# CERALIVE/ceracoder

Hardware: AMD Instinct MI355X
Metric: 1080p H.264 encoded frames/sec per GPU (higher is better)
Workload: dtype u8

## Files before the change

ceracoder_amd/csrc/k_deblock.hip:

```cpp
#include "intra_mb.hpp"

DEV void filter_line(const dev_tables *T, uint8_t *pix, int step, int bS, int qp_p, int qp_q, bool chroma) {
    if (bS == 0) return;
    const int idx = clip3(0, 51, (qp_p + qp_q + 1) >> 1);
    const int alpha = T->alpha[idx], beta = T->beta[idx];
    const int p0 = pix[-step], p1 = pix[-2 * step], q0 = pix[0], q1 = pix[step];
    if (!(iabs(p0 - q0) < alpha && iabs(p1 - p0) < beta && iabs(q1 - q0) < beta)) return;
    if (chroma) {
        if (bS < 4) {
            const int tc = T->tc0[idx][bS - 1] + 1;
            const int dl = clip3(-tc, tc, (((q0 - p0) << 2) + (p1 - q1) + 4) >> 3);
            pix[-step] = (uint8_t)clip255(p0 + dl); pix[0] = (uint8_t)clip255(q0 - dl);
        } else {
            pix[-step] = (uint8_t)((2 * p1 + p0 + q1 + 2) >> 2); pix[0] = (uint8_t)((2 * q1 + q0 + p1 + 2) >> 2);
        }
        return;
    }
    const int p2 = pix[-3 * step], q2 = pix[2 * step];
    const bool ap = iabs(p2 - p0) < beta, aq = iabs(q2 - q0) < beta;
    if (bS < 4) {
        const int tc0 = T->tc0[idx][bS - 1];
        const int tc = tc0 + (ap ? 1 : 0) + (aq ? 1 : 0);
        const int dl = clip3(-tc, tc, (((q0 - p0) << 2) + (p1 - q1) + 4) >> 3);
        pix[-step] = (uint8_t)clip255(p0 + dl); pix[0] = (uint8_t)clip255(q0 - dl);
// ... 228 lines not shown
}
DEV void edge_chroma2(const edge_par &P, int p1, int &p0, int &q0, int q1, int bS) {
    const bool f = (bS != 0) & (adiff(p0, q0) < P.alpha) & (adiff(p1, p0) < P.beta) & (adiff(q1, q0) < P.beta);
    const int tc = (int)((P.tc0 >> (8 * ((bS - 1) & 3))) & 0xFF) + 1;
    const int dl = clip3(-tc, tc, (((q0 - p0) << 2) + (p1 - q1) + 4) >> 3);
    const bool s4 = bS == 4;
    const int sp0 = (2 * p1 + p0 + q1 + 2) >> 2, sq0 = (2 * q1 + q0 + p1 + 2) >> 2, wp0 = clip255(p0 + dl), wq0 = clip255(q0 - dl);
    const int np0 = s4 ? sp0 : wp0, nq0 = s4 ? sq0 : wq0;
    p0 = f ? np0 : p0; q0 = f ? nq0 : q0;
}

DEV int quad_prev(int v) { return __builtin_amdgcn_update_dpp(0, v, 0x90, 0xF, 0xF, false); }
DEV int quad_next(int v) { return __builtin_amdgcn_update_dpp(0, v, 0xF9, 0xF, 0xF, false); }
#define DBT_NB 8
struct dbt_luma { uint8_t t[DBT_NB][256]; uint8_t up[DBT_NB][64]; unsigned par[4][32]; };
struct dbt_chroma { uint8_t t[DBT_NB][128]; uint8_t up[DBT_NB][32]; unsigned par[4][32]; };
DEV uint4 lds128(const void *p) { return *(const uint4 *)p; }

template <bool ALL_INTRA>
DEV void edges4p_luma(const int e, const unsigned par, const bool any4, int *s) {
    int bS = (int)(par & 15u);
    const int alpha = (int)((par >> 8) & 255u), beta = (int)((par >> 16) & 255u), tc0 = (int)(par >> 24);
    if (ALL_INTRA || any4) {
        edge_par PE; PE.alpha = alpha; PE.beta = beta; PE.tc0 = (unsigned)tc0 * 0x010101u;
        edge_luma2<true>(PE, s[0], s[1], s[2], s[3], s[4], s[5], s[6], s[7], e == 0 ? bS : 0, true);
        const int f1 = quad_prev(s[5]), f2 = quad_prev(s[6]);
        s[1] = e == 1 ? f1 : s[1]; s[2] = e == 1 ? f2 : s[2];
        bS = e == 0 ? 0 : bS;
    }
    const int p1 = s[2], p0 = s[3], q0 = s[4], q1 = s[5], q2 = s[6];
    const int mf = ((adiff(p0, q0) - alpha) & (adiff(p1, p0) - beta) & (adiff(q1, q0) - beta) & -bS) >> 31;
// ... 9 lines not shown
    const int np1 = p1 + clip3(-tc0, tc0, (p2 + avg - (p1 << 1)) >> 1);
    s[3] = bsel(mf, clip255(p0 + dl), p0); s[4] = bsel(mf, clip255(q0 - dl), q0);
    s[2] = bsel(mf & map, np1, p1); s[5] = q1f;
}
DEV void edge_chroma_p(const unsigned par, int p1, int &p0, int &q0, int q1) {
    const int bS = (int)(par & 15u), alpha = (int)((par >> 8) & 255u), beta = (int)((par >> 16) & 255u), tc = (int)(par >> 24) + 1;
    const bool f = (bS != 0) & (adiff(p0, q0) < alpha) & (adiff(p1, p0) < beta) & (adiff(q1, q0) < beta);
    const int dl = clip3(-tc, tc, (((q0 - p0) << 2) + (p1 - q1) + 4) >> 3);
    const bool s4 = bS == 4;
    const int sp0 = (2 * p1 + p0 + q1 + 2) >> 2, sq0 = (2 * q1 + q0 + p1 + 2) >> 2, wp0 = clip255(p0 + dl), wq0 = clip255(q0 - dl);
    const int np0 = s4 ? sp0 : wp0, nq0 = s4 ? sq0 : wq0;
    p0 = f ? np0 : p0; q0 = f ? nq0 : q0;
}
DEV unsigned par_word(unsigned nib, unsigned ab, unsigned tcw) { return nib | (ab << 8) | (((tcw >> (8 * ((nib - 1) & 3))) & 255u) << 24); }

template <bool CHROMA, bool ALL_INTRA, int ROWS, bool GATED>
DEV void rows3_body(const db_args &a, const int band, const int nb, uint8_t *lds, const int part) {
    constexpr int rows_mb = CHROMA ? 8 : 16, strip = CHROMA ? 2 : 4, ring_n = CHROMA ? 8 : 16;
    constexpr int ROW_LDS = CHROMA ? (int)sizeof(dbt_chroma) : (int)sizeof(dbt_luma);
    constexpr int TILE = rows_mb * 16, UPB = strip * 16;
    const frame_ctx_t *__restrict__ ctx = &a.ctx;
    const int mbw = ctx->mbw, mbh = ctx->mbh, stride = ctx->stride;
    const int wid = __builtin_amdgcn_readfirstlane(threadIdx.x >> 6), lane = threadIdx.x & 63;
    const int role = wid / ROWS, r = wid - role * ROWS;
    const int my = band * ROWS + r;
    const bool row_ok = my < mbh, last_row = my == mbh - 1 || db_slice_last(ctx, my), dbtop = db_has_top(ctx, my);
    const bool fed = row_ok && r == 0 && dbtop;
    const bool feeds = row_ok && r == ROWS - 1 && !last_row;
    if (!ALL_INTRA && a.row_done) {
        if (threadIdx.x < 64) {
            const int r = (band - 1) * ROWS - 1 + (int)threadIdx.x;
            const bool mine = (int)threadIdx.x < 3 * ROWS + 1 && r >= 0 && r < mbh;
            const unsigned *w = a.row_done + (mine ? r * MI355_PROG_STRIDE : 0);
            int spins = 0;
            while (__ballot(mine && (int)(ld_sc1(w) - a.row_need) < 0)) {
                __builtin_amdgcn_s_sleep(8);
                if (++spins > DB_SPIN_MAX) { st_sc1(a.err, 17u | ((unsigned)band << 8) | (CHROMA ? 0x8000u : 0u)); break; }
                if ((spins & 1023) == 0 && ld_sc1(a.err)) break;
            }
            __builtin_amdgcn_fence(__ATOMIC_ACQUIRE, "agent");
            asm volatile("s_waitcnt vmcnt(0)" ::: "memory");
        }
        __syncthreads();
    }
    if (ALL_INTRA && a.iband_done) {
        if (threadIdx.x == 0) {
            const unsigned tag = ~ctx->epoch;
            const int r_lo = band * ROWS > 0 ? band * ROWS - 1 : 0, r_hi = band * ROWS + ROWS - 1 < mbh ? band * ROWS + ROWS - 1 : mbh - 1;
            int spins = 0;
            for (int ib = r_lo / a.ib_rows; ib <= r_hi / a.ib_rows; ib++)
                while (ld_sc1(a.iband_done + ib) != tag) {
                    __builtin_amdgcn_s_sleep(8);
                    if (++spins > DB_SPIN_MAX) { st_sc1(a.err, 11u); break; } if ((spins & 1023) == 0 && ld_sc1(a.err)) { break; }
                }
            __builtin_amdgcn_fence(__ATOMIC_ACQUIRE, "agent");
            asm volatile("s_waitcnt vmcnt(0)" ::: "memory");
        }
        __syncthreads();
    }
    if (a.qpc) {
        if (threadIdx.x == 0) {
            const unsigned need = a.qpc_base + (unsigned)((band + 1) * ROWS < mbh ? (band + 1) * ROWS : mbh);
            int spins = 0;
            while ((int)(ld_sc1(a.qpc) - need) < 0) {
                __builtin_amdgcn_s_sleep(8);
                if (++spins > DB_SPIN_MAX) { st_sc1(a.err, 23u | ((unsigned)band << 8)); break; }
                if ((spins & 1023) == 0 && ld_sc1(a.err)) break;
            }
            __builtin_amdgcn_fence(__ATOMIC_ACQUIRE, "agent");
            asm volatile("s_waitcnt vmcnt(0)" ::: "memory");
        }
        __syncthreads();
    }
#ifdef TL_PROF
    if (!CHROMA && threadIdx.x == 0) { const int sl = band == 0 ? 9 : band == nb / 2 ? 11 : band == nb - 1 ? 13 : -1; if (sl >= 0) *((volatile unsigned long long *)ctx->dbrec + (ctx->epoch & 63) * 16 + sl) = wall_clock64(); }
#endif
    constexpr int PARW = CHROMA ? 16 : 32;
    unsigned *partab = a.partab + (CHROMA ? (size_t)nb * ROWS * mbw * 32 : 0) + (size_t)band * ROWS * mbw * PARW;
    unsigned *flagw = (unsigned *)(lds + ROWS * ROW_LDS);
    unsigned *firsti = flagw + 4;
    unsigned *busyw = firsti + ROWS;
    if (threadIdx.x < 3) flagw[threadIdx.x] = 0;
    if (threadIdx.x < 2) busyw[threadIdx.x] = 0;
    if (GATED && threadIdx.x < ROWS) firsti[threadIdx.x] = (unsigned)mbw;
    const int cut_mid = mbw >> 1, cut_w = (mbw >> 2) < 31 ? (mbw >> 2) : 31;
    __syncthreads();
    {
        const dev_tables *T = &g_tab;
        const int per = ROWS * mbw;
        for (int j = threadIdx.x; j < per; j += 192 * ROWS) {
            const int row = band * ROWS + j / mbw;
            if (row < mbh) {
                unsigned w[16], pw[PARW];
                const bool work = db_record(ctx, T, j % mbw, row, w);
                if (GATED && (ldg32(&ctx->mbi[(size_t)row * mbw + j % mbw].mb_type) & 255u) != 1u) atomicMin(&firsti[j / mbw], (unsigned)(j % mbw));
#pragma unroll
                for (int d = 0; d < 2; d++)
#pragma unroll
                    for (int ed = 0; ed < (CHROMA ? 2 : 4); ed++)
#pragma unroll
                        for (int sg = 0; sg < 4; sg++) {
                            unsigned nib, ab, tc;
                            if (!CHROMA) {
                                nib = (w[2 * d + (ed >> 1)] >> (16 * (ed & 1) + 4 * sg)) & 15u;
                                ab = ed == 0 ? w[4 + 2 * d] : w[8]; tc = ed == 0 ? w[5 + 2 * d] : w[9];
                            } else {
                                nib = (w[2 * d + ed] >> (4 * sg)) & 15u;
                                ab = ed == 0 ? w[10 + 2 * d] : w[14]; tc = ed == 0 ? w[11 + 2 * d] : w[15];
                            }
                            pw[d * (PARW / 2) + ed * 4 + sg] = par_word(nib, ab, tc);
                        }
#pragma unroll
                for (int q = 0; q < PARW / 4; q++) stg128(partab + (size_t)j * PARW + 4 * q, make_uint4(pw[4 * q], pw[4 * q + 1], pw[4 * q + 2], pw[4 * q + 3]));
                if (work) flagw[1] = 1u;
                if (part >= 0) {
                    const int kc = j % mbw - (cut_mid - cut_w);
                    if (kc >= 0 && kc <= 2 * cut_w && ((pw[0] | pw[1] | pw[2] | pw[3]) & 15u) != 0) atomicOr(&busyw[kc >> 5], 1u << (kc & 31));
                }
            }
        }
#ifdef TL_PROF
        if (!CHROMA && band == 0 && threadIdx.x == 0) *((volatile unsigned long long *)ctx->dbrec + (ctx->epoch & 63) * 16 + 14) = wall_clock64();
#endif
        if (!ALL_INTRA) {
            for (int i = threadIdx.x; i < 2 * per; i += 192 * ROWS) {
                const int which = i < per ? 0 : 2, j = i < per ? i : i - per;
                const int row = (band - 1 + which) * ROWS + j / mbw;
                if (row >= 0 && row < mbh) {
                    const mb_info_t m = ld_mbinfo(&ctx->mbi[(size_t)row * mbw + j % mbw]);
                    if (m.mb_type != 1 || (m.nzmask & 0xFFFFu) != 0) flagw[which] = 1u;
                }
            }
            __syncthreads();
            for (int which = 0; which < 3; which += 2)
                if (flagw[which] == 0)
                    for (int j = threadIdx.x; j < per; j += 192 * ROWS) {
                        const int row = (band - 1 + which) * ROWS + j / mbw;
                        unsigned w[16];
                        if (row >= 0 && row < mbh && db_record(ctx, T, j % mbw, row, w)) flagw[which] = 1u;
                    }
        }
    }
    asm volatile("s_waitcnt vmcnt(0)" ::: "memory");
    __syncthreads();
    auto publish = [&](const bool drained) {
        if (!a.band_done) return;
        if (!drained) { asm volatile("s_waitcnt vmcnt(0)" ::: "memory"); __syncthreads(); }
        if (part >= 0) {
            if (threadIdx.x == 0) {
                __builtin_amdgcn_fence(__ATOMIC_RELEASE, "agent");
                asm volatile("s_waitcnt vmcnt(0)" ::: "memory");
                flagw[3] = __hip_atomic_fetch_add(a.part_cnt + 2 * band + (CHROMA ? 1 : 0), 1u, __ATOMIC_RELAXED, __HIP_MEMORY_SCOPE_AGENT) & 1u;
            }
            __syncthreads();
            if (flagw[3] == 0) return;
        }
        if (threadIdx.x < DB_DONE_COPIES) {
            __builtin_amdgcn_fence(__ATOMIC_RELEASE, "agent");
            asm volatile("s_waitcnt vmcnt(0)" ::: "memory");
            st_sc1(a.band_done + DB_DONE_STRIDE * threadIdx.x + 2 * band + (CHROMA ? 1 : 0), ctx->epoch);
        }
    };
    uint2 *cutg = part >= 0 ? (uint2 *)(a.part_cnt + 2 * nb) + 2 * band + (CHROMA ? 1 : 0) : nullptr;
    if (!ALL_INTRA && flagw[1] == 0) {
        if (cutg && threadIdx.x == 0) st64_sc1(cutg, make_uint2(0u, ctx->epoch));
        publish(true);
        return;
    }
    int x0 = 0, x1 = mbw;
    if (part >= 0) {
        int cut = mbw;
        int cut_up = 0;
        if (!ALL_INTRA && db_has_top(ctx, band * ROWS) && flagw[0] != 0) {
            if (threadIdx.x == 0) {
                uint2 g;
                int spins = 0;
                while ((g = ld64_sc1(cutg - 2)).y != ctx->epoch) {
                    __builtin_amdgcn_s_sleep(4);
                    if (++spins > DB_SPIN_MAX) { st_sc1(a.err, 24u | ((unsigned)band << 8) | (CHROMA ? 0x8000u : 0u)); g.x = 0; break; }
                    if ((spins & 1023) == 0 && ld_sc1(a.err)) { g.x = 0; break; }
                }
                flagw[3] = g.x;
            }
            __syncthreads();
            cut_up = (int)flagw[3];
            __syncthreads();
        }
        if (!ALL_INTRA && mbw >= 16) {
            int tgt = cut_w - (cut_w >> 3);
            const int lo = (cut_up > 0 && cut_up < mbw) ? cut_up - (cut_mid - cut_w) : 0;
            tgt = tgt > lo ? tgt : lo;
            const unsigned long long busy = (unsigned long long)busyw[0] | ((unsigned long long)busyw[1] << 32);
            for (int d = 0; d <= 2 * cut_w && cut == mbw; d++) {
                if (tgt + d <= 2 * cut_w && !((busy >> (tgt + d)) & 1ull)) cut = cut_mid - cut_w + tgt + d;
                else if (tgt - d >= lo && tgt - d >= 0 && !((busy >> (tgt - d)) & 1ull)) cut = cut_mid - cut_w + tgt - d;
            }
        }
        cut = __builtin_amdgcn_readfirstlane(cut);
        if (threadIdx.x == 0) st64_sc1(cutg, make_uint2((unsigned)cut, ctx->epoch));
        if (part == 0) x1 = cut; else x0 = cut;
        if (x0 >= x1) { publish(true); return; }
    }
#ifdef TL_PROF
    if (!CHROMA && band == 0 && threadIdx.x == 0) *((volatile unsigned long long *)ctx->dbrec + (ctx->epoch & 63) * 16 + 15) = wall_clock64();
#endif
    const bool up_work = ALL_INTRA || flagw[0] != 0;
    const bool dn_work = ALL_INTRA || flagw[2] != 0;
    const unsigned epoch = ctx->epoch;
    uint2 *gran_up = a.gran + (CHROMA ? (size_t)nb * mbw * 16 : 0) + (size_t)(band > 0 ? band - 1 : 0) * mbw * ring_n;
    uint2 *gran_my = a.gran + (CHROMA ? (size_t)nb * mbw * 16 : 0) + (size_t)band * mbw * ring_n;
    uint8_t *__restrict__ plane = CHROMA ? ctx->rec_uv : ctx->rec_y;
    const size_t row0 = (size_t)my * rows_mb;
    uint8_t *rowl = lds + r * ROW_LDS;
    uint8_t *tiles = rowl;
    uint8_t *ups = rowl + DBT_NB * TILE;
    unsigned *pars = (unsigned *)(rowl + DBT_NB * (TILE + UPB));
    uint8_t *tiles_up = lds + (r > 0 ? r - 1 : 0) * ROW_LDS;
    const int keep = last_row ? rows_mb : rows_mb - strip;
    const int t_end = (x1 - x0) + ROWS + 1;
    const int k = lane >> 2, e = lane & 3;
    uint4 preA, preB;
    uint2 gA, gB;
    const bool rlane = lane < rows_mb, uplane = lane >= 16 && lane < 16 + strip, glane = lane >= 32 && lane < 32 + ring_n;
    const int my_c = row_ok ? my : mbh - 1;
    constexpr int PL = PARW / 4;
    const bool plane_l = lane >= 16 && lane < 16 + PL;
// ... 9 lines not shown
    unsigned nmiss = 0;
#define DBT_TICK(i) do { tm1 = __builtin_readcyclecounter(); pc[i] += tm1 - tm0; tm0 = tm1; } while (0)
#define DBT_T0() tm0 = __builtin_readcyclecounter()
#else
#define DBT_TICK(i) do { } while (0)
#define DBT_T0() do { } while (0)
#endif
    const int t_last = t_end | 1;
    if (role == 0) {
        for (int t = -2; t <= t_last; t++) {
            DBT_T0();
            const int x = x0 + t - 1 - r;
            const bool act = row_ok && x >= x0 && x < x1;
                uint8_t *tile = tiles + (x & (DBT_NB - 1)) * TILE;
                if (act) {
                    const unsigned par = pars[(x & 3) * PARW + (CHROMA ? (lane & 1) * 4 + (lane >> 3) : e * 4 + (k >> 2))];
                    if (!CHROMA) {
                        uint8_t *tl = tiles + ((x - 1) & (DBT_NB - 1)) * TILE;
                        unsigned *pw = (unsigned *)(e == 0 ? tl + k * 16 + 12 : tile + k * 16 + 4 * e - 4), *qw = (unsigned *)(tile + k * 16 + 4 * e);
                        const unsigned w0 = *pw, w1 = *qw;
                        const unsigned long long work = __ballot((par & 15u) != 0);
                        if (ALL_INTRA || work) {
                            int s[8];
#pragma unroll
                            for (int i = 0; i < 4; i++) { s[i] = byte_of(w0, i); s[4 + i] = byte_of(w1, i); }
                            edges4p_luma<ALL_INTRA>(e, par, __ballot((par & 15u) == 4u) != 0, s);
                            const int nx = quad_next(s[2] | (s[3] << 8));
                            const unsigned hi = e == 3 ? (unsigned)(s[6] | (s[7] << 8)) : (unsigned)nx;
                            *qw = (unsigned)s[4] | ((unsigned)s[5] << 8) | (hi << 16);
                            if (e == 0 && x > x0) *pw = pack4(s[0], s[1], s[2], s[3]);
                        }
                    } else if (lane < 32) {
                        const int kk = lane >> 2, c = (lane >> 1) & 1, ee = lane & 1;
                        uint8_t *tl = tiles + ((x - 1) & (DBT_NB - 1)) * TILE;
                        uint8_t *pb = ee == 0 ? tl + kk * 16 + 12 + c : tile + kk * 16 + 4 + c, *qb = tile + kk * 16 + 8 * ee + c;
                        int p1 = pb[0], p0 = pb[2], q0 = qb[0], q1 = qb[2];
                        edge_chroma_p(par, p1, p0, q0, q1);
                        if (ee != 0 || x > x0) pb[2] = (uint8_t)p0;
                        qb[0] = (uint8_t)q0;
                    }
                }
                DBT_TICK(0);
                BAND_BARRIER();
                DBT_TICK(1);
                if (act) {
                    const unsigned par = pars[(x & 3) * PARW + PARW / 2 + (CHROMA ? (lane & 1) * 4 + (lane >> 3) : e * 4 + (k >> 2))];
                    uint8_t *upb = fed ? ups + (x & (DBT_NB - 1)) * UPB : tiles_up + (x & (DBT_NB - 1)) * TILE + (rows_mb - strip) * 16;
                    if (!CHROMA) {
                        uint8_t *pb = (e == 0 ? upb : tile + (4 * e - 4) * 16) + k, *qb = tile + 4 * e * 16 + k;
                        int s[8];
#pragma unroll
                        for (int i = 0; i < 4; i++) { s[i] = pb[i * 16]; s[4 + i] = qb[i * 16]; }
                        const unsigned long long work = __ballot((par & 15u) != 0);
                        if (ALL_INTRA || work) {
                            const bool any4 = __ballot((par & 15u) == 4u) != 0;
                            edges4p_luma<ALL_INTRA>(e, par, any4, s);
                            if (e != 0 || dbtop) { pb[2 * 16] = (uint8_t)s[2]; pb[3 * 16] = (uint8_t)s[3]; }
                            qb[0] = (uint8_t)s[4]; qb[16] = (uint8_t)s[5];
                            if ((ALL_INTRA || any4) && e == 0 && dbtop) pb[16] = (uint8_t)s[1];
                        }
                    } else if (lane < 32) {
                        const int kb = lane >> 1, ee = lane & 1;
                        uint8_t *pb = (ee == 0 ? upb : tile + 2 * 16) + kb, *qb = tile + 4 * ee * 16 + kb;
                        int p1 = pb[0], p0 = pb[16], q0 = qb[0], q1 = qb[16];
                        edge_chroma_p(par, p1, p0, q0, q1);
                        if (ee != 0 || dbtop) pb[16] = (uint8_t)p0;
                        qb[0] = (uint8_t)q0;
                    }
                }
            DBT_TICK(2);
        }
    } else if (role == 1) {
        int fin = GATED ? (int)firsti[r] : 0x7FFF;
        auto mstep = [&](const int t, uint4 &cur, uint2 &gpre) __attribute__((always_inline)) {
            DBT_T0();
            const int x = x0 + t - 1 - r;
            const bool act = row_ok && x >= x0 && x < x1;
                const int xm = x + 1, xl = x + 3;
                const bool lands = row_ok && xm >= x0 && xm < x1;
                if (lands) {
                    if (rlane) *(uint4 *)(tiles + (xm & (DBT_NB - 1)) * TILE + lane * 16) = cur;
                    if (plane_l) *(uint4 *)(pars + (xm & 3) * PARW + 4 * (lane - 16)) = cur;
                }
                if (fed && act) {
                    unsigned *dst = (unsigned *)(ups + (x & (DBT_NB - 1)) * UPB) + gj;
                    const bool late = up_work && __ballot(glane && gpre.y != epoch) != 0;
                    if (glane) *dst = gpre.x;
                    if (late) {
                        uint2 g2;
                        int spins = 0;
#ifdef DBT_PROF
                        nmiss++;
#endif
                        do {
                            __builtin_amdgcn_s_sleep(1);
                            g2 = ld64_sc1(gran_up + (size_t)x * ring_n + gj);
                            if (++spins > DB_SPIN_MAX) { st_sc1(a.err, 12u | ((unsigned)band << 8) | (CHROMA ? 0x8000u : 0u) | ((unsigned)x << 16) | ((unsigned)((__ballot(glane && g2.y == epoch) >> 32) & 0xFu) << 28)); break; } if ((spins & 1023) == 0 && ld_sc1(a.err)) { break; }
                        } while (__ballot(glane && g2.y != epoch));
                        if (glane) *dst = g2.x;
                    }
                }
                DBT_TICK(0);
                BAND_BARRIER();
                DBT_TICK(1);
                {
                    const int xg = x + 2, xgc = xg < 0 ? 0 : (xg < mbw ? xg : mbw - 1), xlc = xl < 0 ? 0 : (xl < mbw ? xl : mbw - 1);
                    const int need = xl + 2 < mbw ? xl + 2 : mbw;
                    if (GATED && row_ok && xl >= x0 && xl < x1 && fin < need) {
                        const unsigned tag = (epoch & 0xFFFFFu) << 12;
                        int spins = 0;
                        for (;;) {
                            const unsigned v = (unsigned)__builtin_amdgcn_readfirstlane((int)ld_sc1(a.ip_progress + my * MI355_PROG_STRIDE));
// ... 37 lines not shown
            DBT_TICK(2);
        }
    }
    if (a.band_done) {
#ifdef DBG_DELAY_BAND
        if (band == DBG_DELAY_BAND) {
            for (int i = 0; i < 100; i++) __builtin_amdgcn_s_sleep(127);
            if (role == 2 && row_ok && lane < keep)
                for (int xs2 = mbw - 4 > 0 ? mbw - 4 : 0; xs2 < mbw; xs2++) stg128(st_ptr + xs2 * 16, lds128(tiles + (xs2 & (DBT_NB - 1)) * TILE + lane * 16));
        }
#endif
        publish(false);
    }
    tl_last(ctx, 8);
#ifdef TL_PROF
    if (!CHROMA && threadIdx.x == 0) { const int sl = band == 0 ? 10 : band == nb / 2 ? 12 : -1; if (sl >= 0) *((volatile unsigned long long *)ctx->dbrec + (ctx->epoch & 63) * 16 + sl) = wall_clock64(); }
#endif
#ifdef DBT_PROF
    if (lane == 0 && band < 2) {
        unsigned *o = (unsigned *)(ctx->dbrec) + (CHROMA ? 128 : 0) + 64 * band + 16 * r + 4 * role;
        for (int i = 0; i < 3; i++) o[i] = (unsigned)pc[i];
        o[3] = (unsigned)(t_last + 3) | (nmiss << 16);
    }
#endif
}

template <int NW>
DEV void qp_chain_rows(const db_args &a) {
    __shared__ int row_last[NW], row_in[NW];
    const frame_ctx_t *__restrict__ ctx = &a.ctx;
    const int mbw = ctx->mbw, mbh = ctx->mbh, lane = threadIdx.x & 63, w = __builtin_amdgcn_readfirstlane(threadIdx.x >> 6);
    const unsigned tag = ~ctx->epoch;
    int carry = ctx->qp;
    for (int r0 = 0; r0 < mbh; r0 += NW) {
        const int r = r0 + w;
        const bool mine = r < mbh;
        if (mine && lane == 0) {
            int spins = 0;
            if (!ctx->all_intra && a.row_done)
// ... 80 lines not shown
            __syncthreads();
            if (threadIdx.x == 0) {
                __builtin_amdgcn_fence(__ATOMIC_RELEASE, "agent");
                asm volatile("s_waitcnt vmcnt(0)" ::: "memory");
                __hip_atomic_fetch_add(a.ip_done, 1u, __ATOMIC_RELAXED, __HIP_MEMORY_SCOPE_AGENT);
            }
            return;
        }
        bi -= a.nip; nwg -= a.nip;
    }
    if (bi == 0) tl_first(&a.ctx, 7);
    if (a.started && threadIdx.x == 0) __hip_atomic_fetch_add(a.started, 1u, __ATOMIC_RELAXED, __HIP_MEMORY_SCOPE_AGENT);
    int part = -1;
    if (!ALL_INTRA && a.part_cnt) { part = bi & 1; bi >>= 1; nwg >>= 1; }
    const int nl = nwg >> 1;
    if (bi < nl) rows3_body<false, ALL_INTRA, ROWS, GATED>(a, a.band0 + bi, a.nb_total, lds, part);
    else rows3_body<true, ALL_INTRA, ROWS, GATED>(a, a.band0 + bi - nl, a.nb_total, lds, part);
}

int k_deblock_diags(int mbw, int mbh) { return mbw + 2 * (mbh - 1); }
void k_launch_deblock_diag(const frame_ctx_t *d_ctx, int mbw, int mbh, int diag, hipStream_t s) {
    int y_lo = diag - (mbw - 1);
    y_lo = y_lo > 0 ? (y_lo + 1) >> 1 : 0;
    int y_hi = diag / 2 < mbh - 1 ? diag / 2 : mbh - 1;
    if (y_hi < y_lo) return;
    hipLaunchKernelGGL(deblock_kernel, dim3(y_hi - y_lo + 1), dim3(64), 0, s, d_ctx, diag);
}
#ifndef DB_ROWS
#define DB_ROWS MI355_BAND_ROWS
#endif
int k_deblock_bands16(int mbh) { return (mbh + DB_ROWS - 1) / DB_ROWS; }
size_t k_deblock_gran_bytes(int mbw, int mbh) { return (size_t)k_deblock_bands16(mbh) * mbw * 24 * sizeof(uint2); }
__global__ __launch_bounds__(64) void wait_started_kernel(const unsigned *started, unsigned count, unsigned *err) {
    if (threadIdx.x) return;
    int spins = 0;
    while ((int)(ld_sc1(started) - count) < 0) {
        __builtin_amdgcn_s_sleep(32);
        if (++spins > DB_SPIN_MAX) { st_sc1(err, 4u); break; }
        if ((spins & 255) == 0 && ld_sc1(err)) break;
    }
}
void k_launch_wait_started(const unsigned *d_started, unsigned count, unsigned *d_err, hipStream_t s) { hipLaunchKernelGGL(wait_started_kernel, dim3(1), dim3(64), 0, s, d_started, count, d_err); }
size_t k_deblock_done_bytes(void) { return (size_t)DB_DONE_COPIES * DB_DONE_STRIDE * sizeof(unsigned); }
size_t k_deblock_partab_bytes(int mbw, int mbh) { return (size_t)k_deblock_bands16(mbh) * DB_ROWS * mbw * 48 * sizeof(unsigned); }
size_t k_deblock_part_bytes(int mbh) {
#ifdef DBG_DELAY_BAND
    (void)mbh; return 0;
#else
    return 6 * (size_t)k_deblock_bands16(mbh) * sizeof(unsigned);
#endif
}
int k_launch_deblock_bands(const frame_ctx_t *h_ctx, const db_launch_t *l, hipStream_t s) {
    static_assert(DB_ROWS == MI355_BAND_ROWS, "db_launch_wgs() and pmb_kernel's gate count bands of MI355_BAND_ROWS rows");
    constexpr size_t lds = (size_t)DB_ROWS * sizeof(dbt_luma) + 16 + 4 * DB_ROWS + 8;
    static_assert(lds <= 48 * 1024, "above 48 KB of dynamic LDS every instantiation launched here would need hipFuncAttributeMaxDynamicSharedMemorySize");
    const bool follows = l->variant == DB_P_FOLLOWS_IP || l->variant == DB_P_FUSED_IP, fused = l->variant == DB_P_FUSED_IP;
    if (!l->err || !l->gran || !l->partab || (follows && !l->ip_progress) || (fused && (!l->ip_strips || !l->ip_done || !l->row_done)) ||
        (l->parts && (!l->part_cnt || l->variant == DB_ALL_INTRA)) || (l->qpc && !l->qpc_word)) return -1;
    const int mbh = h_ctx->mbh;
    db_args a;
    a.ctx = *h_ctx; a.err = l->err; a.band0 = 0; a.nb_total = k_deblock_bands16(mbh); a.gran = (uint2 *)l->gran; a.ip_progress = follows ? l->ip_progress : nullptr; a.partab = l->partab; a.iband_done = l->iband_done; a.ib_rows = l->ib_rows > 0 ? l->ib_rows : DB_ROWS; a.band_done = l->band_done; a.started = l->started; a.row_done = l->row_done; a.row_need = l->row_need;
    a.nip = fused ? mbh : 0; a.ip_progress_w = fused ? l->ip_progress : nullptr; a.ip_strips = fused ? l->ip_strips : nullptr; a.ip_done = fused ? l->ip_done : nullptr;
    a.qpc = l->qpc ? l->qpc_word : nullptr; a.qpc_base = l->qpc_base;
    a.part_cnt = l->parts ? l->part_cnt : nullptr;
    const dim3 grid(db_launch_wgs(mbh, l->variant, l->parts, l->qpc).grid), block(192 * DB_ROWS);
    switch (l->variant) {
    case DB_ALL_INTRA: hipLaunchKernelGGL((deblock_rows3_kernel<DB_ROWS, true, false, false>), grid, block, lds, s, a); break;
    case DB_P: hipLaunchKernelGGL((deblock_rows3_kernel<DB_ROWS, false, false, false>), grid, block, lds, s, a); break;
    case DB_P_FOLLOWS_IP: hipLaunchKernelGGL((deblock_rows3_kernel<DB_ROWS, false, true, false>), grid, block, lds, s, a); break;
    case DB_P_FUSED_IP: hipLaunchKernelGGL((deblock_rows3_kernel<DB_ROWS, false, true, true>), grid, block, lds, s, a); break;
    default: return -1;
    }
    return 0;
}
// ... 1 lines not shown
```

Measured before the change: 7438.

## Replace wavefront-pipelined chroma deblock with phase-parallel band body

Chroma deblocking no longer goes through the templated per-row LDS-tile wavefront pipeline shared with luma. It now runs a dedicated band body that computes the edge parameters, then filters in whole-band phases (vertical edges, horizontal edges) directly in global memory, with block-wide barriers between phases. The split-part path for chroma is reduced to a publish-only workgroup, and the wait and publish logic is factored into shared helpers. This is meant to remove per-macroblock pipeline synchronisation for the lighter chroma plane, at the cost of more global memory traffic and full-block barriers, and with the split-part work for chroma no longer shared across workgroups.

```diff
diff --git a/ceracoder_amd/csrc/k_deblock.hip b/ceracoder_amd/csrc/k_deblock.hip
--- a/ceracoder_amd/csrc/k_deblock.hip
+++ b/ceracoder_amd/csrc/k_deblock.hip
@@ -266,7 +266,6 @@
 DEV int quad_next(int v) { return __builtin_amdgcn_update_dpp(0, v, 0xF9, 0xF, 0xF, false); }
 #define DBT_NB 8
 struct dbt_luma { uint8_t t[DBT_NB][256]; uint8_t up[DBT_NB][64]; unsigned par[4][32]; };
-struct dbt_chroma { uint8_t t[DBT_NB][128]; uint8_t up[DBT_NB][32]; unsigned par[4][32]; };
 DEV uint4 lds128(const void *p) { return *(const uint4 *)p; }
 
 template <bool ALL_INTRA>
@@ -306,10 +305,87 @@
 }
 DEV unsigned par_word(unsigned nib, unsigned ab, unsigned tcw) { return nib | (ab << 8) | (((tcw >> (8 * ((nib - 1) & 3))) & 255u) << 24); }
 
-template <bool CHROMA, bool ALL_INTRA, int ROWS, bool GATED>
+#ifdef TL_PROF
+DEV void tl_plane_end(const frame_ctx_t *ctx, const int my0, const int plane) {
+    if (threadIdx.x) return;
+    const int sl = ctx->slice_dbf == 2 && ctx->slice_rows > 0 ? my0 / ctx->slice_rows : 0;
+    atomicMax((unsigned long long *)ctx->dbrec + 64 * 16 + (ctx->epoch & 63) * 16 + 2 * (sl < 7 ? sl : 7) + plane, (unsigned long long)wall_clock64());
+}
+#endif
+template <bool ALL_INTRA, int ROWS>
+DEV void band_wait_inputs(const db_args &a, const int band, const bool chroma) {
+    const frame_ctx_t *__restrict__ ctx = &a.ctx;
+    const int mbh = ctx->mbh;
+    if (!ALL_INTRA && a.row_done) {
+        if (threadIdx.x < 64) {
+            const int r = (band - 1) * ROWS - 1 + (int)threadIdx.x;
+            const bool mine = (int)threadIdx.x < 3 * ROWS + 1 && r >= 0 && r < mbh;
+            const unsigned *w = a.row_done + (mine ? r * MI355_PROG_STRIDE : 0);
+            int spins = 0;
+            while (__ballot(mine && (int)(ld_sc1(w) - a.row_need) < 0)) {
+                __builtin_amdgcn_s_sleep(8);
+                if (++spins > DB_SPIN_MAX) { st_sc1(a.err, 17u | ((unsigned)band << 8) | (chroma ? 0x8000u : 0u)); break; }
+                if ((spins & 1023) == 0 && ld_sc1(a.err)) break;
+            }
+            __builtin_amdgcn_fence(__ATOMIC_ACQUIRE, "agent");
+            asm volatile("s_waitcnt vmcnt(0)" ::: "memory");
+        }
+        __syncthreads();
+    }
+    if (ALL_INTRA && a.iband_done) {
+        if (threadIdx.x == 0) {
+            const unsigned tag = ~ctx->epoch;
+            const int r_lo = band * ROWS > 0 ? band * ROWS - 1 : 0, r_hi = band * ROWS + ROWS - 1 < mbh ? band * ROWS + ROWS - 1 : mbh - 1;
+            int spins = 0;
+            for (int ib = r_lo / a.ib_rows; ib <= r_hi / a.ib_rows; ib++)
+                while (ld_sc1(a.iband_done + ib) != tag) {
+                    __builtin_amdgcn_s_sleep(8);
+                    if (++spins > DB_SPIN_MAX) { st_sc1(a.err, 11u); break; } if ((spins & 1023) == 0 && ld_sc1(a.err)) { break; }
+                }
+            __builtin_amdgcn_fence(__ATOMIC_ACQUIRE, "agent");
+            asm volatile("s_waitcnt vmcnt(0)" ::: "memory");
+        }
+        __syncthreads();
+    }
+    if (a.qpc) {
+        if (threadIdx.x == 0) {
+            const unsigned need = a.qpc_base + (unsigned)((band + 1) * ROWS < mbh ? (band + 1) * ROWS : mbh);
+            int spins = 0;
+            while ((int)(ld_sc1(a.qpc) - need) < 0) {
+                __builtin_amdgcn_s_sleep(8);
+                if (++spins > DB_SPIN_MAX) { st_sc1(a.err, 23u | ((unsigned)band << 8)); break; }
+                if ((spins & 1023) == 0 && ld_sc1(a.err)) break;
+            }
+            __builtin_amdgcn_fence(__ATOMIC_ACQUIRE, "agent");
+            asm volatile("s_waitcnt vmcnt(0)" ::: "memory");
+        }
+        __syncthreads();
+    }
+}
+
+DEV void band_publish(const db_args &a, const int band, const bool chroma, const int part, unsigned *hs, const bool drained) {
+    if (!a.band_done) return;
+    if (!drained) { asm volatile("s_waitcnt vmcnt(0)" ::: "memory"); __syncthreads(); }
+    if (part >= 0) {
+        if (threadIdx.x == 0) {
+            __builtin_amdgcn_fence(__ATOMIC_RELEASE, "agent");
+            asm volatile("s_waitcnt vmcnt(0)" ::: "memory");
+            *hs = __hip_atomic_fetch_add(a.part_cnt + 2 * band + (chroma ? 1 : 0), 1u, __ATOMIC_RELAXED, __HIP_MEMORY_SCOPE_AGENT) & 1u;
+        }
+        __syncthreads();
+        if (*hs == 0) return;
+    }
+    if (threadIdx.x < DB_DONE_COPIES) {
+        __builtin_amdgcn_fence(__ATOMIC_RELEASE, "agent");
+        asm volatile("s_waitcnt vmcnt(0)" ::: "memory");
+        st_sc1(a.band_done + DB_DONE_STRIDE * threadIdx.x + 2 * band + (chroma ? 1 : 0), a.ctx.epoch);
+    }
+}
+
+template <bool ALL_INTRA, int ROWS, bool GATED>
 DEV void rows3_body(const db_args &a, const int band, const int nb, uint8_t *lds, const int part) {
-    constexpr int rows_mb = CHROMA ? 8 : 16, strip = CHROMA ? 2 : 4, ring_n = CHROMA ? 8 : 16;
-    constexpr int ROW_LDS = CHROMA ? (int)sizeof(dbt_chroma) : (int)sizeof(dbt_luma);
+    constexpr int rows_mb = 16, strip = 4, ring_n = 16;
+    constexpr int ROW_LDS = (int)sizeof(dbt_luma);
     constexpr int TILE = rows_mb * 16, UPB = strip * 16;
     const frame_ctx_t *__restrict__ ctx = &a.ctx;
     const int mbw = ctx->mbw, mbh = ctx->mbh, stride = ctx->stride;
@@ -319,56 +395,12 @@
     const bool row_ok = my < mbh, last_row = my == mbh - 1 || db_slice_last(ctx, my), dbtop = db_has_top(ctx, my);
     const bool fed = row_ok && r == 0 && dbtop;
     const bool feeds = row_ok && r == ROWS - 1 && !last_row;
-    if (!ALL_INTRA && a.row_done) {
-        if (threadIdx.x < 64) {
-            const int r = (band - 1) * ROWS - 1 + (int)threadIdx.x;
-            const bool mine = (int)threadIdx.x < 3 * ROWS + 1 && r >= 0 && r < mbh;
-            const unsigned *w = a.row_done + (mine ? r * MI355_PROG_STRIDE : 0);
-            int spins = 0;
-            while (__ballot(mine && (int)(ld_sc1(w) - a.row_need) < 0)) {
-                __builtin_amdgcn_s_sleep(8);
-                if (++spins > DB_SPIN_MAX) { st_sc1(a.err, 17u | ((unsigned)band << 8) | (CHROMA ? 0x8000u : 0u)); break; }
-                if ((spins & 1023) == 0 && ld_sc1(a.err)) break;
-            }
-            __builtin_amdgcn_fence(__ATOMIC_ACQUIRE, "agent");
-            asm volatile("s_waitcnt vmcnt(0)" ::: "memory");
-        }
-        __syncthreads();
-    }
-    if (ALL_INTRA && a.iband_done) {
-        if (threadIdx.x == 0) {
-            const unsigned tag = ~ctx->epoch;
-            const int r_lo = band * ROWS > 0 ? band * ROWS - 1 : 0, r_hi = band * ROWS + ROWS - 1 < mbh ? band * ROWS + ROWS - 1 : mbh - 1;
-            int spins = 0;
-            for (int ib = r_lo / a.ib_rows; ib <= r_hi / a.ib_rows; ib++)
-                while (ld_sc1(a.iband_done + ib) != tag) {
-                    __builtin_amdgcn_s_sleep(8);
-                    if (++spins > DB_SPIN_MAX) { st_sc1(a.err, 11u); break; } if ((spins & 1023) == 0 && ld_sc1(a.err)) { break; }
-                }
-            __builtin_amdgcn_fence(__ATOMIC_ACQUIRE, "agent");
-            asm volatile("s_waitcnt vmcnt(0)" ::: "memory");
-        }
-        __syncthreads();
-    }
-    if (a.qpc) {
-        if (threadIdx.x == 0) {
-            const unsigned need = a.qpc_base + (unsigned)((band + 1) * ROWS < mbh ? (band + 1) * ROWS : mbh);
-            int spins = 0;
-            while ((int)(ld_sc1(a.qpc) - need) < 0) {
-                __builtin_amdgcn_s_sleep(8);
-                if (++spins > DB_SPIN_MAX) { st_sc1(a.err, 23u | ((unsigned)band << 8)); break; }
-                if ((spins & 1023) == 0 && ld_sc1(a.err)) break;
-            }
-            __builtin_amdgcn_fence(__ATOMIC_ACQUIRE, "agent");
-            asm volatile("s_waitcnt vmcnt(0)" ::: "memory");
-        }
-        __syncthreads();
-    }
+    band_wait_inputs<ALL_INTRA, ROWS>(a, band, false);
 #ifdef TL_PROF
-    if (!CHROMA && threadIdx.x == 0) { const int sl = band == 0 ? 9 : band == nb / 2 ? 11 : band == nb - 1 ? 13 : -1; if (sl >= 0) *((volatile unsigned long long *)ctx->dbrec + (ctx->epoch & 63) * 16 + sl) = wall_clock64(); }
-#endif
-    constexpr int PARW = CHROMA ? 16 : 32;
-    unsigned *partab = a.partab + (CHROMA ? (size_t)nb * ROWS * mbw * 32 : 0) + (size_t)band * ROWS * mbw * PARW;
+    if (threadIdx.x == 0) { const int sl = band == 0 ? 9 : band == nb / 2 ? 11 : band == nb - 1 ? 13 : -1; if (sl >= 0) *((volatile unsigned long long *)ctx->dbrec + (ctx->epoch & 63) * 16 + sl) = wall_clock64(); }
+#endif
+    constexpr int PARW = 32;
+    unsigned *partab = a.partab + (size_t)band * ROWS * mbw * PARW;
     unsigned *flagw = (unsigned *)(lds + ROWS * ROW_LDS);
     unsigned *firsti = flagw + 4;
     unsigned *busyw = firsti + ROWS;
@@ -389,18 +421,11 @@
 #pragma unroll
                 for (int d = 0; d < 2; d++)
 #pragma unroll
-                    for (int ed = 0; ed < (CHROMA ? 2 : 4); ed++)
+                    for (int ed = 0; ed < 4; ed++)
 #pragma unroll
                         for (int sg = 0; sg < 4; sg++) {
-                            unsigned nib, ab, tc;
-                            if (!CHROMA) {
-                                nib = (w[2 * d + (ed >> 1)] >> (16 * (ed & 1) + 4 * sg)) & 15u;
-                                ab = ed == 0 ? w[4 + 2 * d] : w[8]; tc = ed == 0 ? w[5 + 2 * d] : w[9];
-                            } else {
-                                nib = (w[2 * d + ed] >> (4 * sg)) & 15u;
-                                ab = ed == 0 ? w[10 + 2 * d] : w[14]; tc = ed == 0 ? w[11 + 2 * d] : w[15];
-                            }
-                            pw[d * (PARW / 2) + ed * 4 + sg] = par_word(nib, ab, tc);
+                            const unsigned nib = (w[2 * d + (ed >> 1)] >> (16 * (ed & 1) + 4 * sg)) & 15u;
+                            pw[d * (PARW / 2) + ed * 4 + sg] = par_word(nib, ed == 0 ? w[4 + 2 * d] : w[8], ed == 0 ? w[5 + 2 * d] : w[9]);
                         }
 #pragma unroll
                 for (int q = 0; q < PARW / 4; q++) stg128(partab + (size_t)j * PARW + 4 * q, make_uint4(pw[4 * q], pw[4 * q + 1], pw[4 * q + 2], pw[4 * q + 3]));
@@ -412,7 +437,7 @@
             }
         }
 #ifdef TL_PROF
-        if (!CHROMA && band == 0 && threadIdx.x == 0) *((volatile unsigned long long *)ctx->dbrec + (ctx->epoch & 63) * 16 + 14) = wall_clock64();
+        if (band == 0 && threadIdx.x == 0) *((volatile unsigned long long *)ctx->dbrec + (ctx->epoch & 63) * 16 + 14) = wall_clock64();
 #endif
         if (!ALL_INTRA) {
             for (int i = threadIdx.x; i < 2 * per; i += 192 * ROWS) {
@@ -435,27 +460,11 @@
     }
     asm volatile("s_waitcnt vmcnt(0)" ::: "memory");
     __syncthreads();
-    auto publish = [&](const bool drained) {
-        if (!a.band_done) return;
-        if (!drained) { asm volatile("s_waitcnt vmcnt(0)" ::: "memory"); __syncthreads(); }
-        if (part >= 0) {
-            if (threadIdx.x == 0) {
-                __builtin_amdgcn_fence(__ATOMIC_RELEASE, "agent");
-                asm volatile("s_waitcnt vmcnt(0)" ::: "memory");
-                flagw[3] = __hip_atomic_fetch_add(a.part_cnt + 2 * band + (CHROMA ? 1 : 0), 1u, __ATOMIC_RELAXED, __HIP_MEMORY_SCOPE_AGENT) & 1u;
-            }
-            __syncthreads();
-            if (flagw[3] == 0) return;
-        }
-        if (threadIdx.x < DB_DONE_COPIES) {
-            __builtin_amdgcn_fence(__ATOMIC_RELEASE, "agent");
-            asm volatile("s_waitcnt vmcnt(0)" ::: "memory");
-            st_sc1(a.band_done + DB_DONE_STRIDE * threadIdx.x + 2 * band + (CHROMA ? 1 : 0), ctx->epoch);
-        }
-    };
-    uint2 *cutg = part >= 0 ? (uint2 *)(a.part_cnt + 2 * nb) + 2 * band + (CHROMA ? 1 : 0) : nullptr;
+    auto publish = [&](const bool drained) { band_publish(a, band, false, part, flagw + 3, drained); };
+    uint2 *cutg = part >= 0 ? (uint2 *)(a.part_cnt + 2 * nb) + 2 * band : nullptr;
+    auto leave_cut = [&](const unsigned col) { const uint2 g = make_uint2(col, ctx->epoch); st64_sc1(cutg, g); st64_sc1(cutg + 1, g); };
     if (!ALL_INTRA && flagw[1] == 0) {
-        if (cutg && threadIdx.x == 0) st64_sc1(cutg, make_uint2(0u, ctx->epoch));
+        if (cutg && threadIdx.x == 0) leave_cut(0u);
         publish(true);
         return;
     }
@@ -469,7 +478,7 @@
                 int spins = 0;
                 while ((g = ld64_sc1(cutg - 2)).y != ctx->epoch) {
                     __builtin_amdgcn_s_sleep(4);
-                    if (++spins > DB_SPIN_MAX) { st_sc1(a.err, 24u | ((unsigned)band << 8) | (CHROMA ? 0x8000u : 0u)); g.x = 0; break; }
+                    if (++spins > DB_SPIN_MAX) { st_sc1(a.err, 24u | ((unsigned)band << 8)); g.x = 0; break; }
                     if ((spins & 1023) == 0 && ld_sc1(a.err)) { g.x = 0; break; }
                 }
                 flagw[3] = g.x;
@@ -489,19 +498,19 @@
             }
         }
         cut = __builtin_amdgcn_readfirstlane(cut);
-        if (threadIdx.x == 0) st64_sc1(cutg, make_uint2((unsigned)cut, ctx->epoch));
+        if (threadIdx.x == 0) leave_cut((unsigned)cut);
         if (part == 0) x1 = cut; else x0 = cut;
         if (x0 >= x1) { publish(true); return; }
     }
 #ifdef TL_PROF
-    if (!CHROMA && band == 0 && threadIdx.x == 0) *((volatile unsigned long long *)ctx->dbrec + (ctx->epoch & 63) * 16 + 15) = wall_clock64();
+    if (band == 0 && threadIdx.x == 0) *((volatile unsigned long long *)ctx->dbrec + (ctx->epoch & 63) * 16 + 15) = wall_clock64();
 #endif
     const bool up_work = ALL_INTRA || flagw[0] != 0;
     const bool dn_work = ALL_INTRA || flagw[2] != 0;
     const unsigned epoch = ctx->epoch;
-    uint2 *gran_up = a.gran + (CHROMA ? (size_t)nb * mbw * 16 : 0) + (size_t)(band > 0 ? band - 1 : 0) * mbw * ring_n;
-    uint2 *gran_my = a.gran + (CHROMA ? (size_t)nb * mbw * 16 : 0) + (size_t)band * mbw * ring_n;
-    uint8_t *__restrict__ plane = CHROMA ? ctx->rec_uv : ctx->rec_y;
+    uint2 *gran_up = a.gran + (size_t)(band > 0 ? band - 1 : 0) * mbw * ring_n;
+    uint2 *gran_my = a.gran + (size_t)band * mbw * ring_n;
+    uint8_t *__restrict__ plane = ctx->rec_y;
     const size_t row0 = (size_t)my * rows_mb;
     uint8_t *rowl = lds + r * ROW_LDS;
     uint8_t *tiles = rowl;
@@ -541,58 +550,39 @@
             const bool act = row_ok && x >= x0 && x < x1;
                 uint8_t *tile = tiles + (x & (DBT_NB - 1)) * TILE;
                 if (act) {
-                    const unsigned par = pars[(x & 3) * PARW + (CHROMA ? (lane & 1) * 4 + (lane >> 3) : e * 4 + (k >> 2))];
-                    if (!CHROMA) {
-                        uint8_t *tl = tiles + ((x - 1) & (DBT_NB - 1)) * TILE;
-                        unsigned *pw = (unsigned *)(e == 0 ? tl + k * 16 + 12 : tile + k * 16 + 4 * e - 4), *qw = (unsigned *)(tile + k * 16 + 4 * e);
-                        const unsigned w0 = *pw, w1 = *qw;
-                        const unsigned long long work = __ballot((par & 15u) != 0);
-                        if (ALL_INTRA || work) {
-                            int s[8];
-#pragma unroll
-                            for (int i = 0; i < 4; i++) { s[i] = byte_of(w0, i); s[4 + i] = byte_of(w1, i); }
-                            edges4p_luma<ALL_INTRA>(e, par, __ballot((par & 15u) == 4u) != 0, s);
-                            const int nx = quad_next(s[2] | (s[3] << 8));
-                            const unsigned hi = e == 3 ? (unsigned)(s[6] | (s[7] << 8)) : (unsigned)nx;
-                            *qw = (unsigned)s[4] | ((unsigned)s[5] << 8) | (hi << 16);
-                            if (e == 0 && x > x0) *pw = pack4(s[0], s[1], s[2], s[3]);
-                        }
-                    } else if (lane < 32) {
-                        const int kk = lane >> 2, c = (lane >> 1) & 1, ee = lane & 1;
-                        uint8_t *tl = tiles + ((x - 1) & (DBT_NB - 1)) * TILE;
-                        uint8_t *pb = ee == 0 ? tl + kk * 16 + 12 + c : tile + kk * 16 + 4 + c, *qb = tile + kk * 16 + 8 * ee + c;
-                        int p1 = pb[0], p0 = pb[2], q0 = qb[0], q1 = qb[2];
-                        edge_chroma_p(par, p1, p0, q0, q1);
-                        if (ee != 0 || x > x0) pb[2] = (uint8_t)p0;
-                        qb[0] = (uint8_t)q0;
+                    const unsigned par = pars[(x & 3) * PARW + e * 4 + (k >> 2)];
+                    uint8_t *tl = tiles + ((x - 1) & (DBT_NB - 1)) * TILE;
+                    unsigned *pw = (unsigned *)(e == 0 ? tl + k * 16 + 12 : tile + k * 16 + 4 * e - 4), *qw = (unsigned *)(tile + k * 16 + 4 * e);
+                    const unsigned w0 = *pw, w1 = *qw;
+                    const unsigned long long work = __ballot((par & 15u) != 0);
+                    if (ALL_INTRA || work) {
+                        int s[8];
+#pragma unroll
+                        for (int i = 0; i < 4; i++) { s[i] = byte_of(w0, i); s[4 + i] = byte_of(w1, i); }
+                        edges4p_luma<ALL_INTRA>(e, par, __ballot((par & 15u) == 4u) != 0, s);
+                        const int nx = quad_next(s[2] | (s[3] << 8));
+                        const unsigned hi = e == 3 ? (unsigned)(s[6] | (s[7] << 8)) : (unsigned)nx;
+                        *qw = (unsigned)s[4] | ((unsigned)s[5] << 8) | (hi << 16);
+                        if (e == 0 && x > x0) *pw = pack4(s[0], s[1], s[2], s[3]);
                     }
                 }
                 DBT_TICK(0);
                 BAND_BARRIER();
                 DBT_TICK(1);
                 if (act) {
-                    const unsigned par = pars[(x & 3) * PARW + PARW / 2 + (CHROMA ? (lane & 1) * 4 + (lane >> 3) : e * 4 + (k >> 2))];
+                    const unsigned par = pars[(x & 3) * PARW + PARW / 2 + e * 4 + (k >> 2)];
                     uint8_t *upb = fed ? ups + (x & (DBT_NB - 1)) * UPB : tiles_up + (x & (DBT_NB - 1)) * TILE + (rows_mb - strip) * 16;
-                    if (!CHROMA) {
-                        uint8_t *pb = (e == 0 ? upb : tile + (4 * e - 4) * 16) + k, *qb = tile + 4 * e * 16 + k;
-                        int s[8];
-#pragma unroll
-                        for (int i = 0; i < 4; i++) { s[i] = pb[i * 16]; s[4 + i] = qb[i * 16]; }
-                        const unsigned long long work = __ballot((par & 15u) != 0);
-                        if (ALL_INTRA || work) {
-                            const bool any4 = __ballot((par & 15u) == 4u) != 0;
-                            edges4p_luma<ALL_INTRA>(e, par, any4, s);
-                            if (e != 0 || dbtop) { pb[2 * 16] = (uint8_t)s[2]; pb[3 * 16] = (uint8_t)s[3]; }
-                            qb[0] = (uint8_t)s[4]; qb[16] = (uint8_t)s[5];
-                            if ((ALL_INTRA || any4) && e == 0 && dbtop) pb[16] = (uint8_t)s[1];
-                        }
-                    } else if (lane < 32) {
-                        const int kb = lane >> 1, ee = lane & 1;
-                        uint8_t *pb = (ee == 0 ? upb : tile + 2 * 16) + kb, *qb = tile + 4 * ee * 16 + kb;
-                        int p1 = pb[0], p0 = pb[16], q0 = qb[0], q1 = qb[16];
-                        edge_chroma_p(par, p1, p0, q0, q1);
-                        if (ee != 0 || dbtop) pb[16] = (uint8_t)p0;
-                        qb[0] = (uint8_t)q0;
+                    uint8_t *pb = (e == 0 ? upb : tile + (4 * e - 4) * 16) + k, *qb = tile + 4 * e * 16 + k;
+                    int s[8];
+#pragma unroll
+                    for (int i = 0; i < 4; i++) { s[i] = pb[i * 16]; s[4 + i] = qb[i * 16]; }
+                    const unsigned long long work = __ballot((par & 15u) != 0);
+                    if (ALL_INTRA || work) {
+                        const bool any4 = __ballot((par & 15u) == 4u) != 0;
+                        edges4p_luma<ALL_INTRA>(e, par, any4, s);
+                        if (e != 0 || dbtop) { pb[2 * 16] = (uint8_t)s[2]; pb[3 * 16] = (uint8_t)s[3]; }
+                        qb[0] = (uint8_t)s[4]; qb[16] = (uint8_t)s[5];
+                        if ((ALL_INTRA || any4) && e == 0 && dbtop) pb[16] = (uint8_t)s[1];
                     }
                 }
             DBT_TICK(2);
@@ -622,7 +612,7 @@
                         do {
                             __builtin_amdgcn_s_sleep(1);
                             g2 = ld64_sc1(gran_up + (size_t)x * ring_n + gj);
-                            if (++spins > DB_SPIN_MAX) { st_sc1(a.err, 12u | ((unsigned)band << 8) | (CHROMA ? 0x8000u : 0u) | ((unsigned)x << 16) | ((unsigned)((__ballot(glane && g2.y == epoch) >> 32) & 0xFu) << 28)); break; } if ((spins & 1023) == 0 && ld_sc1(a.err)) { break; }
+                            if (++spins > DB_SPIN_MAX) { st_sc1(a.err, 12u | ((unsigned)band << 8) | ((unsigned)x << 16) | ((unsigned)((__ballot(glane && g2.y == epoch) >> 32) & 0xFu) << 28)); break; } if ((spins & 1023) == 0 && ld_sc1(a.err)) { break; }
                         } while (__ballot(glane && g2.y != epoch));
                         if (glane) *dst = g2.x;
                     }
@@ -690,15 +680,175 @@
     }
     tl_last(ctx, 8);
 #ifdef TL_PROF
-    if (!CHROMA && threadIdx.x == 0) { const int sl = band == 0 ? 10 : band == nb / 2 ? 12 : -1; if (sl >= 0) *((volatile unsigned long long *)ctx->dbrec + (ctx->epoch & 63) * 16 + sl) = wall_clock64(); }
+    if (threadIdx.x == 0) { const int sl = band == 0 ? 10 : band == nb / 2 ? 12 : -1; if (sl >= 0) *((volatile unsigned long long *)ctx->dbrec + (ctx->epoch & 63) * 16 + sl) = wall_clock64(); }
+    tl_plane_end(ctx, band * ROWS, 0);
 #endif
 #ifdef DBT_PROF
     if (lane == 0 && band < 2) {
-        unsigned *o = (unsigned *)(ctx->dbrec) + (CHROMA ? 128 : 0) + 64 * band + 16 * r + 4 * role;
+        unsigned *o = (unsigned *)(ctx->dbrec) + 64 * band + 16 * r + 4 * role;
         for (int i = 0; i < 3; i++) o[i] = (unsigned)pc[i];
         o[3] = (unsigned)(t_last + 3) | (nmiss << 16);
     }
 #endif
+}
+
+DEV void chroma_vedge(uint8_t *q, const unsigned par) {
+    if ((par & 15u) == 0) return;
+    const unsigned wp = ldg32(q - 4), wq = ldg32(q);
+    int p0u = byte_of(wp, 2), p0v = byte_of(wp, 3), q0u = byte_of(wq, 0), q0v = byte_of(wq, 1);
+    edge_chroma_p(par, byte_of(wp, 0), p0u, q0u, byte_of(wq, 2));
+    edge_chroma_p(par, byte_of(wp, 1), p0v, q0v, byte_of(wq, 3));
+    stg32(q - 4, (wp & 0xFFFFu) | ((unsigned)p0u << 16) | ((unsigned)p0v << 24));
+    stg32(q, (wq & 0xFFFF0000u) | (unsigned)q0u | ((unsigned)q0v << 8));
+}
+DEV void chroma_hedge(uint8_t *q, const int stride, const unsigned par) {
+    if ((par & 15u) == 0) return;
+    const unsigned w1 = ldg32(q - 2 * stride), w0 = ldg32(q - stride), v0 = ldg32(q), v1 = ldg32(q + stride);
+    unsigned np = 0, nq = 0;
+#pragma unroll
+    for (int c = 0; c < 4; c++) {
+        int p0 = byte_of(w0, c), q0 = byte_of(v0, c);
+        edge_chroma_p(par, byte_of(w1, c), p0, q0, byte_of(v1, c));
+        np |= (unsigned)p0 << (8 * c); nq |= (unsigned)q0 << (8 * c);
+    }
+    stg32(q - stride, np); stg32(q, nq);
+}
+#define CHROMA_PHASE_BARRIER() do { asm volatile("s_waitcnt vmcnt(0)" ::: "memory"); __syncthreads(); } while (0)
+
+template <bool ALL_INTRA, int ROWS, bool GATED>
+DEV void chroma_band_body(const db_args &a, const int band, const int nb, uint8_t *lds, const int part) {
+    constexpr int NT = 192 * ROWS;
+    const frame_ctx_t *__restrict__ ctx = &a.ctx;
+    const int mbw = ctx->mbw, mbh = ctx->mbh, stride = ctx->stride;
+    unsigned *flagw = (unsigned *)lds;
+    unsigned *firsti = flagw + 4;
+    unsigned *upv = firsti + 1 + ROWS;
+    if (part == 1) { band_publish(a, band, true, part, flagw + 3, true); return; }
+    band_wait_inputs<ALL_INTRA, ROWS>(a, band, true);
+    const int my0 = band * ROWS, rows = mbh - my0 < ROWS ? mbh - my0 : ROWS;
+    const bool dbtop = db_has_top(ctx, my0);
+    const bool last_row = my0 + rows == mbh || db_slice_last(ctx, my0 + rows - 1);
+    const int r_lo = dbtop ? -1 : 0;
+    if (threadIdx.x == 0) flagw[0] = 0;
+    if (GATED && threadIdx.x <= ROWS) firsti[threadIdx.x] = (unsigned)mbw;
+    __syncthreads();
+    unsigned *partab = a.partab + (size_t)nb * ROWS * mbw * 32 + (size_t)band * ROWS * mbw * 16;
+    {
+        const dev_tables *T = &g_tab;
+        for (int j = threadIdx.x; j < (rows - r_lo) * mbw; j += NT) {
+            const int jr = j / mbw, mx = j - jr * mbw, rr = jr + r_lo, row = my0 + rr;
+            unsigned w[16], any = 0;
+            db_record(ctx, T, mx, row, w);
+            if (GATED && (ldg32(&ctx->mbi[(size_t)row * mbw + mx].mb_type) & 255u) != 1u) atomicMin(&firsti[rr + 1], (unsigned)mx);
+            if (rr < 0) {
+                const unsigned n0 = (w[0] >> 12) & 15u, n1 = (w[1] >> 12) & 15u;
+                upv[2 * mx] = par_word(n0, w[10], w[11]); upv[2 * mx + 1] = par_word(n1, w[14], w[15]);
+                any = n0 | n1;
+            } else {
+                unsigned pw[16];
+#pragma unroll
+                for (int d = 0; d < 2; d++)
+#pragma unroll
+                    for (int ed = 0; ed < 2; ed++)
+#pragma unroll
+                        for (int sg = 0; sg < 4; sg++) {
+                            const unsigned nib = (w[2 * d + ed] >> (4 * sg)) & 15u;
+                            pw[d * 8 + ed * 4 + sg] = par_word(nib, ed == 0 ? w[10 + 2 * d] : w[14], ed == 0 ? w[11 + 2 * d] : w[15]);
+                            any |= nib;
+                        }
+#pragma unroll
+                for (int q = 0; q < 4; q++) stg128(partab + (size_t)(rr * mbw + mx) * 16 + 4 * q, make_uint4(pw[4 * q], pw[4 * q + 1], pw[4 * q + 2], pw[4 * q + 3]));
+            }
+            if (any) flagw[0] = 1u;
+        }
+    }
+    CHROMA_PHASE_BARRIER();
+    if (flagw[0] == 0) { band_publish(a, band, true, part, flagw + 3, true); return; }
+    if (GATED) {
+        if (threadIdx.x < 64) {
+            const int i = (int)threadIdx.x;
+            const bool mine = i <= ROWS && firsti[i <= ROWS ? i : 0] < (unsigned)mbw;
+            const unsigned *w = a.ip_progress + (size_t)(mine ? my0 - 1 + i : 0) * MI355_PROG_STRIDE;
+            const unsigned tag = IP_EPOCH(ctx->epoch);
+            int spins = 0;
+            for (;;) {
+                const unsigned v = ld_sc1(w);
+                if (!__ballot(mine && !((v & ~0xFFFu) == tag && (int)(v & 0xFFFu) >= mbw))) break;
+                __builtin_amdgcn_s_sleep(8);
+                if (++spins > DB_SPIN_MAX) { st_sc1(a.err, 25u | ((unsigned)band << 8) | 0x8000u); break; }
+                if ((spins & 1023) == 0 && ld_sc1(a.err)) break;
+            }
+            __builtin_amdgcn_fence(__ATOMIC_ACQUIRE, "agent");
+            asm volatile("s_waitcnt vmcnt(0)" ::: "memory");
+        }
+        __syncthreads();
+    }
+    uint8_t *__restrict__ plane = ctx->rec_uv;
+    const int ne = 2 * mbw;
+#ifdef DBT_PROF
+    unsigned long long tm[5];
+    tm[0] = __builtin_readcyclecounter();
+#define CPH_TICK(i) tm[i] = __builtin_readcyclecounter()
+#else
+#define CPH_TICK(i) do { } while (0)
+#endif
+    {
+        const int n = ((last_row ? rows : rows - 1) - r_lo) * 2 * ne;
+        for (int i = threadIdx.x; i < n; i += NT) {
+            const int lr = i / ne, e = i - lr * ne, rr = r_lo + (lr >> 1);
+            if (e == 0) continue;
+            const unsigned par = rr < 0 ? upv[e] : ldg32(partab + (size_t)(rr * mbw + (e >> 1)) * 16 + (e & 1) * 4 + 3);
+            chroma_vedge(plane + ((size_t)(my0 + rr) * 8 + 6 + (lr & 1)) * stride + 8 * e, par);
+        }
+    }
+    CHROMA_PHASE_BARRIER();
+    CPH_TICK(1);
+    auto hphase = [&](const bool right) __attribute__((always_inline)) {
+        const int n = rows * 2 * mbw * (right ? 1 : 4);
+        for (int i = threadIdx.x; i < n; i += NT) {
+            const int dw = right ? 3 : (i & 3), t = right ? i : (i >> 2);
+            if (!right && dw == 3) continue;
+            const int re = t / mbw, mx = t - re * mbw, rr = re >> 1, ee = re & 1, row = my0 + rr;
+            if (ee == 0 && !db_has_top(ctx, row)) continue;
+            const unsigned par = ldg32(partab + (size_t)(rr * mbw + mx) * 16 + 8 + ee * 4 + dw);
+            chroma_hedge(plane + ((size_t)row * 8 + 4 * ee) * stride + 16 * mx + 4 * dw, stride, par);
+        }
+    };
+    hphase(true);
+    CHROMA_PHASE_BARRIER();
+    CPH_TICK(2);
+    {
+        const int n = rows * 6 * ne;
+        for (int i = threadIdx.x; i < n; i += NT) {
+            const int lr = i / ne, e = i - lr * ne, rr = lr / 6, line = lr - 6 * rr;
+            if (e == 0) continue;
+            const unsigned par = ldg32(partab + (size_t)(rr * mbw + (e >> 1)) * 16 + (e & 1) * 4 + (line >> 1));
+            chroma_vedge(plane + ((size_t)(my0 + rr) * 8 + line) * stride + 8 * e, par);
+        }
+    }
+    CHROMA_PHASE_BARRIER();
+    CPH_TICK(3);
+#ifdef DBG_DELAY_BAND
+    if (band == DBG_DELAY_BAND) for (int i = 0; i < 100; i++) __builtin_amdgcn_s_sleep(127);
+#endif
+    hphase(false);
+    band_publish(a, band, true, part, flagw + 3, false);
+    tl_last(ctx, 8);
+#ifdef TL_PROF
+    tl_plane_end(ctx, my0, 1);
+#endif
+#ifdef DBT_PROF
+    if (threadIdx.x == 0 && band < 2) {
+        CPH_TICK(4);
+        unsigned *o = (unsigned *)(ctx->dbrec) + 128 + 64 * band;
+        for (int i = 0; i < 4; i++)
+            for (int role = 0; role < 3; role++) {
+                o[16 * i + 4 * role] = role == 0 ? (unsigned)(tm[i + 1] - tm[i]) : 0u;
+                o[16 * i + 4 * role + 1] = 0u; o[16 * i + 4 * role + 2] = 0u; o[16 * i + 4 * role + 3] = 1u;
+            }
+    }
+#endif
+#undef CPH_TICK
 }
 
 template <int NW>
@@ -809,8 +959,8 @@
     int part = -1;
     if (!ALL_INTRA && a.part_cnt) { part = bi & 1; bi >>= 1; nwg >>= 1; }
     const int nl = nwg >> 1;
-    if (bi < nl) rows3_body<false, ALL_INTRA, ROWS, GATED>(a, a.band0 + bi, a.nb_total, lds, part);
-    else rows3_body<true, ALL_INTRA, ROWS, GATED>(a, a.band0 + bi - nl, a.nb_total, lds, part);
+    if (bi < nl) rows3_body<ALL_INTRA, ROWS, GATED>(a, a.band0 + bi, a.nb_total, lds, part);
+    else chroma_band_body<ALL_INTRA, ROWS, GATED>(a, a.band0 + bi - nl, a.nb_total, lds, part);
 }
 
 int k_deblock_diags(int mbw, int mbh) { return mbw + 2 * (mbh - 1); }
@@ -825,7 +975,7 @@
 #define DB_ROWS MI355_BAND_ROWS
 #endif
 int k_deblock_bands16(int mbh) { return (mbh + DB_ROWS - 1) / DB_ROWS; }
-size_t k_deblock_gran_bytes(int mbw, int mbh) { return (size_t)k_deblock_bands16(mbh) * mbw * 24 * sizeof(uint2); }
+size_t k_deblock_gran_bytes(int mbw, int mbh) { return (size_t)k_deblock_bands16(mbh) * mbw * 16 * sizeof(uint2); }
 __global__ __launch_bounds__(64) void wait_started_kernel(const unsigned *started, unsigned count, unsigned *err) {
     if (threadIdx.x) return;
     int spins = 0;
@@ -853,6 +1003,7 @@
     if (!l->err || !l->gran || !l->partab || (follows && !l->ip_progress) || (fused && (!l->ip_strips || !l->ip_done || !l->row_done)) ||
         (l->parts && (!l->part_cnt || l->variant == DB_ALL_INTRA)) || (l->qpc && !l->qpc_word)) return -1;
     const int mbh = h_ctx->mbh;
+    if ((size_t)(5 + DB_ROWS + 2 * h_ctx->mbw) * sizeof(unsigned) > lds) return -1;
     db_args a;
     a.ctx = *h_ctx; a.err = l->err; a.band0 = 0; a.nb_total = k_deblock_bands16(mbh); a.gran = (uint2 *)l->gran; a.ip_progress = follows ? l->ip_progress : nullptr; a.partab = l->partab; a.iband_done = l->iband_done; a.ib_rows = l->ib_rows > 0 ? l->ib_rows : DB_ROWS; a.band_done = l->band_done; a.started = l->started; a.row_done = l->row_done; a.row_need = l->row_need;
     a.nip = fused ? mbh : 0; a.ip_progress_w = fused ? l->ip_progress : nullptr; a.ip_strips = fused ? l->ip_strips : nullptr; a.ip_done = fused ? l->ip_done : nullptr;
```

New measurement: 7364. 0.99x the previous value.
